# barrust/pyprobables

Measured on AMD Instinct MI355X. Metric: million keys/sec insert+lookup (Bloom m=2^28 k=7, CMS 2^20x5), higher is better.
Workload: dtype u64; 1 GPU; cfg2 Bloom m=2^28 k=7: per rank per step clear + insert 10M 16B keys + (merge) + check them; keys_per_rank=10000000, key_bytes=16, m_bits=268435456, k=7, parallelism=single GPU

## Files before the change

include/psk.h:

```cpp
#ifndef PSK_H
#define PSK_H

#include <stdint.h>

#ifdef __cplusplus
extern "C" {
#endif

typedef struct psk_sketch psk_sketch;

enum psk_status {
    PSK_OK = 0,
    PSK_EINVAL = -1,
    PSK_ENODEV = -2,
    PSK_ENOMEM = -3,
    PSK_EHIP = -4,
    PSK_ECONTRACT = -5
};

enum psk_where {
    PSK_HOST = 0,
    PSK_DEVICE = 1,
    PSK_DEVICE_BORROWED = 2
};

enum psk_layout { PSK_KEYS_FIXED = 0, PSK_KEYS_VARLEN8 = 1, PSK_KEYS_VARLEN32 = 2, PSK_KEYS_HASHES = 3 };

enum psk_query { PSK_Q_MIN = 0, PSK_Q_MEAN = 1, PSK_Q_MEANMIN = 2 };

enum psk_kind { PSK_KIND_BLOOM = 0, PSK_KIND_CBF = 1, PSK_KIND_CMS = 2 };

enum psk_opmode { PSK_OP_ADD = 0, PSK_OP_REMOVE = 1, PSK_OP_SIGNED = 2  };

enum psk_counter {
    PSK_CTR_ADDED = 0,
    PSK_CTR_REMOVED = 1,
    PSK_CTR_VIOLATIONS = 2,
    PSK_CTR_SATURATED = 3,
    PSK_CTR_ABS_BOUND = 4,
    PSK_CTR_COUNT = 8
};

const char *psk_last_error(void);
int psk_version(void);
int psk_device_count(int *count);
int psk_set_option(const char *name, int64_t value);
int psk_get_option(const char *name, int64_t *value);
int psk_sketch_set_option(psk_sketch *s, const char *name, int64_t value);
int psk_sketch_get_option(psk_sketch *s, const char *name, int64_t *value);
int psk_debug_phase_profile(psk_sketch *s, uint32_t nbuckets, uint32_t nwg, uint64_t out[12]);

uint64_t psk_bloom_table_bytes(uint64_t m_bits);
uint64_t psk_cbf_table_bytes(uint64_t m);
uint64_t psk_cms_table_bytes(uint64_t width, uint32_t depth);
int psk_bloom_create(uint64_t m_bits, uint32_t k, int device, void *ext_table, psk_sketch **out);
int psk_cbf_create(uint64_t m, uint32_t k, int device, void *ext_table, psk_sketch **out);
int psk_cms_create(uint64_t width, uint32_t depth, int device, void *ext_table, psk_sketch **out);
int psk_destroy(psk_sketch *s);
int psk_clear(psk_sketch *s, void *stream);
int psk_synchronize(psk_sketch *s, void *stream);
int psk_release_scratch(psk_sketch *s);
int psk_scratch_bytes(psk_sketch *s, uint64_t bytes[3]);
int psk_table_info(psk_sketch *s, void **dev_ptr, uint64_t *padded_bytes, uint64_t *logical_bytes);
int psk_read_table(psk_sketch *s, void *dst_host, uint64_t nbytes, void *stream);
int psk_write_table(psk_sketch *s, const void *src_host, uint64_t nbytes, void *stream);
int psk_get_counters(psk_sketch *s, int64_t out[PSK_CTR_COUNT], void *stream);
int psk_reset_counters(psk_sketch *s, void *stream);
int psk_rescan_bound(psk_sketch *s, void *stream);

int psk_bloom_add(psk_sketch *s, int layout, const void *data, const uint64_t *offsets, uint64_t n,
                  uint32_t key_len, int where, void *stream);
int psk_bloom_check(psk_sketch *s, int layout, const void *data, const uint64_t *offsets, uint64_t n,
                    uint32_t key_len, int where, uint8_t *out, void *stream);
int psk_bloom_check_bits(psk_sketch *s, int layout, const void *data, const uint64_t *offsets, uint64_t n,
                         uint32_t key_len, int where, uint64_t *out_bits, uint64_t *hits, void *stream);
int psk_bloom_check_begin(psk_sketch *s, int layout, const void *data, const uint64_t *offsets, uint64_t n, uint32_t key_len,
                          void *stream);
int psk_bloom_check_finish(psk_sketch *s, uint8_t *out_dev, void *stream);

int psk_cbf_add(psk_sketch *s, int layout, const void *data, const uint64_t *offsets, uint64_t n,
                uint32_t key_len, const uint32_t *weights, int where, void *stream);
int psk_cbf_remove(psk_sketch *s, int layout, const void *data, const uint64_t *offsets, uint64_t n,
                   uint32_t key_len, const uint32_t *weights, int where, void *stream);
int psk_cbf_check(psk_sketch *s, int layout, const void *data, const uint64_t *offsets, uint64_t n,
                  uint32_t key_len, int where, uint32_t *out, void *stream);
int psk_cbf_update_combined(psk_sketch *s, int layout, const void *data, const uint64_t *offsets, uint64_t n,
                            uint32_t key_len, const uint32_t *weights, int remove, int where, void *stream);
int psk_flush(psk_sketch *s, void *stream);
int psk_cbf_update_ordered(psk_sketch *s, int layout, const void *data, const uint64_t *offsets, uint64_t n,
                           uint32_t key_len, const int64_t *weights, int opmode, int where, uint32_t *out,
                           void *stream);

// ... 111 lines not shown
```

pyprobables_amd/_native.py:

```python

from __future__ import annotations

import ctypes as C
import os
from pathlib import Path

from .exceptions import NativeLibraryError

PSK_OK, PSK_EINVAL, PSK_ENODEV, PSK_ENOMEM, PSK_EHIP, PSK_ECONTRACT = 0, -1, -2, -3, -4, -5
HOST, DEVICE, DEVICE_BORROWED = 0, 1, 2
KEYS_FIXED, KEYS_VARLEN8, KEYS_VARLEN32, KEYS_HASHES = 0, 1, 2, 3
Q_MIN, Q_MEAN, Q_MEANMIN = 0, 1, 2
OP_ADD, OP_REMOVE, OP_SIGNED = 0, 1, 2
CTR_ADDED, CTR_REMOVED, CTR_VIOLATIONS, CTR_SATURATED, CTR_ABS_BOUND, CTR_ELS_OUT, CTR_COUNT = 0, 1, 2, 3, 4, 5, 8

LIB_PATH = Path(os.environ.get("PSK_LIB_PATH") or (Path(__file__).resolve().parent / "csrc" / "libpsk_hip.so"))

_vp, _u64, _u32, _i64, _int = C.c_void_p, C.c_uint64, C.c_uint32, C.c_int64, C.c_int
_KEYS = [_int, _vp, _vp, _u64, _u32]

PROTOTYPES = {
    "psk_last_error": (C.c_char_p, []),
    "psk_version": (_int, []),
    "psk_device_count": (_int, [C.POINTER(_int)]),
    "psk_set_option": (_int, [C.c_char_p, _i64]),
    "psk_get_option": (_int, [C.c_char_p, C.POINTER(_i64)]),
    "psk_debug_phase_profile": (_int, [_vp, _u32, _u32, C.POINTER(_u64)]),
    "psk_bloom_table_bytes": (_u64, [_u64]),
    "psk_cbf_table_bytes": (_u64, [_u64]),
    "psk_cms_table_bytes": (_u64, [_u64, _u32]),
    "psk_bloom_create": (_int, [_u64, _u32, _int, _vp, C.POINTER(_vp)]),
    "psk_cbf_create": (_int, [_u64, _u32, _int, _vp, C.POINTER(_vp)]),
    "psk_cms_create": (_int, [_u64, _u32, _int, _vp, C.POINTER(_vp)]),
    "psk_destroy": (_int, [_vp]),
    "psk_clear": (_int, [_vp, _vp]),
    "psk_synchronize": (_int, [_vp, _vp]),
    "psk_table_info": (_int, [_vp, C.POINTER(_vp), C.POINTER(_u64), C.POINTER(_u64)]),
    "psk_read_table": (_int, [_vp, _vp, _u64, _vp]),
    "psk_write_table": (_int, [_vp, _vp, _u64, _vp]),
    "psk_get_counters": (_int, [_vp, C.POINTER(_i64), _vp]),
    "psk_reset_counters": (_int, [_vp, _vp]),
    "psk_rescan_bound": (_int, [_vp, _vp]),
    "psk_sketch_set_option": (_int, [_vp, C.c_char_p, _i64]),
    "psk_sketch_get_option": (_int, [_vp, C.c_char_p, C.POINTER(_i64)]),
    "psk_bloom_add": (_int, [_vp, *_KEYS, _int, _vp]),
    "psk_bloom_check": (_int, [_vp, *_KEYS, _int, _vp, _vp]),
    "psk_bloom_check_begin": (_int, [_vp, *_KEYS, _vp]),
    "psk_bloom_check_finish": (_int, [_vp, _vp, _vp]),
    "psk_bloom_check_bits": (_int, [_vp, *_KEYS, _int, _vp, _vp, _vp]),
    "psk_cbf_add": (_int, [_vp, *_KEYS, _vp, _int, _vp]),
    "psk_cbf_remove": (_int, [_vp, *_KEYS, _vp, _int, _vp]),
    "psk_cbf_check": (_int, [_vp, *_KEYS, _int, _vp, _vp]),
    "psk_cbf_update_combined": (_int, [_vp, *_KEYS, _vp, _int, _int, _vp]),
    "psk_flush": (_int, [_vp, _vp]),
    "psk_cbf_update_ordered": (_int, [_vp, *_KEYS, _vp, _int, _int, _vp, _vp]),
    "psk_cms_add": (_int, [_vp, *_KEYS, _vp, _int, _vp]),
    "psk_cms_remove": (_int, [_vp, *_KEYS, _vp, _int, _vp]),
    "psk_cms_check": (_int, [_vp, *_KEYS, _int, _int, _vp, _vp]),
    "psk_cms_check_meanmin": (_int, [_vp, *_KEYS, _int, _i64, _vp, _vp]),
    "psk_cms_update_ordered": (_int, [_vp, *_KEYS, _vp, _int, _int, _i64, _int, _vp, _vp]),
    "psk_cms_add_running": (_int, [_vp, *_KEYS, _vp, _int, _int, _i64, _vp, _vp, _vp]),
    "psk_cms_update_running": (_int, [_vp, *_KEYS, _vp, _int, _int, _i64, _vp, _vp, _vp]),
    "psk_fnv1a_hash": (_int, [*_KEYS, _u32, _int, _vp, _int, _vp]),
    "psk_digest_chain": (_int, [_int, *_KEYS, _u32, _int, _vp, _int, _vp]),
    "psk_qf_hash": (_int, [*_KEYS, _int, _vp, _int, _vp]),
    "psk_qf_build": (_int, [_u32, _vp, _u64, _vp, _vp, _vp, _vp, _vp, _int, _vp]),
    "psk_qf_check": (_int, [_u32, _vp, _vp, _vp, _vp, *_KEYS, _int, _vp, _int, _vp]),
# ... 126 lines not shown
```

pyprobables_amd/csrc/psk_host.hpp:

```cpp
#pragma once
#include "psk_device.hpp"
#include "psk_partition.hpp"
#include "psk_part_bins.hpp"

#include <hip/hip_runtime.h>

#include <cstdarg>
#include <cstdio>
#include <cstdlib>
#include <cstring>
#include <new>
#include <type_traits>
#include <vector>

#include "../../include/psk.h"

using namespace psk;

#define PSK_HIDDEN __attribute__((visibility("hidden")))

PSK_HIDDEN int fail(int code, const char *fmt, ...);

#define HIP_TRY(expr)                                                                                   \
    do {                                                                                                \
// ... 227 lines not shown
    if (!nib_geometry(s->m, true, g)) return false;
    g->k = s->k;
    g->nwg = 256;
    g->append = 1;
    g->tile = 0;
    const double tile_keys = 2048.0 * 7.0 / (double)(s->k < 1 ? 1 : s->k);
    const double mean = (double)cap * s->k / ((double)g->nbuckets * g->nwg);
    const double runs = 2.0 * (double)cap / (tile_keys * g->nwg) + 64.0;
    const double segcap = mean / 6.0 + 0.5 * runs + 8.0 * __builtin_sqrt(mean) / 6.0 + 16.0;
    if (segcap >= (double)(1u << 24) || (double)g->nbuckets * segcap >= 4294967296.0) return false;
    g->segcap = (uint32_t)segcap;
    return true;
}

PSK_HIDDEN int raise_dyn_lds(const void *kernel, size_t bytes);

template <class K>
static int set_dyn_lds(K kernel, size_t bytes)
{
    return raise_dyn_lds((const void *)kernel, bytes);
}

template <class Pay, int KT, int NT>
static size_t scatter_lds_bytes(const PartGeom *g, uint64_t tile = 0, bool sorted = false)
{
    if (sorted) return scatter_lds_bytes<Pay, KT, NT>(g, tile, false) + 16 + 8 * (size_t)kSortBins + 18 * (size_t)PartTile<Pay, KT, NT>::TILE;
    using Tile = PartTile<Pay, KT, NT>;
    const uint32_t kk = g->k < (uint32_t)KT ? g->k : (uint32_t)KT;
    const size_t tk = tile ? (size_t)tile : (size_t)Tile::TILE;
    const size_t stage_cap = ((tk * kk + (size_t)(Tile::GS - 1) * g->nbuckets) + 3) & ~(size_t)3;
    const size_t stage_words = stage_cap + (Tile::pair ? stage_cap / Tile::GS + 4 : 0);
    return (5 * (size_t)g->nbuckets + 16 + 24 + stage_words) * 4;
}

struct ScatterTarget {
    uint32_t *cnt;
    uint4 *part;
};

#ifndef PSK_LOOKUP_FAT_SLICES
#define PSK_LOOKUP_FAT_SLICES 900
#endif
constexpr uint32_t kLookupFatSlices = PSK_LOOKUP_FAT_SLICES;
constexpr size_t kScatterLdsBudget = 160 * 1024;
constexpr size_t kScatterLdsTwoPerCu = 78 * 1024;

template <class Src>
struct src_fat512 { static constexpr bool value = std::is_same<Src, KeysFixed16>::value || std::is_same<Src, KeysFixed16Multi>::value || std::is_same<Src, KeysFixed8>::value; };

template <class Src, class Pay, int KT>
struct bins_eligible {
    static constexpr bool value = pay_bins_ok<Pay>::value && KT <= 8 && src_fat512<Src>::value;
};
constexpr size_t kBinSlackWords = 8 + 16;
struct BinsPlan {
    uint32_t tile, cap, stride, per_cu;
    size_t lds;
};
template <int KT>
static bool bins_plan(const PartGeom *g, BinsPlan *p)
{
    if (g_part_bins == 0 || g->nbuckets > (uint32_t)kBinThreads * kBinSlicesPerLane || g->nbuckets < 2) return false;
    constexpr double kSigmas = 3.5;
    const uint32_t kk = g->k < (uint32_t)KT ? g->k : (uint32_t)KT;
    p->tile = (uint32_t)kBinThreads * kBinKpt;
    const double mean = (double)p->tile * kk / (double)g->nbuckets;
    uint32_t cap = (uint32_t)(mean + kSigmas * __builtin_sqrt(mean) + 2.0);
    cap = (cap + 5) / 6 * 6;
    p->cap = cap;
    uint32_t stride = kBinHead + cap + 1;
    while (stride % 4 != 2) ++stride;
    p->stride = stride;
    p->lds = ((size_t)g->nbuckets * stride + kBinSlackWords) * 4;
    if (p->lds > kScatterLdsBudget / 2) return false;
    uint32_t per_cu = (uint32_t)(kScatterLdsBudget / p->lds);
    const uint32_t by_waves = 2048u / (uint32_t)kBinThreads;
    p->per_cu = per_cu > by_waves ? by_waves : per_cu;
    return true;
}

template <class Src, class IdxFn, class Pay, class Spill, int KT>
static int launch_scatter_bins(psk_sketch *s, const Src &src, const IdxFn &idxfn, const Pay &pay, const Spill &spill, PartGeom *g, uint64_t n,
                               hipStream_t st, uint32_t want_wgs, const BinsPlan &bp)
{
    const uint32_t kk = g->k < (uint32_t)KT ? g->k : (uint32_t)KT;
    const uint64_t tile_full = bp.tile;
    const uint64_t ntiles = (n + tile_full - 1) / tile_full;
    uint64_t nwg = 256ULL * bp.per_cu;
    if (want_wgs) nwg = want_wgs;
    if (nwg > 64u * kApplyWaves) nwg = 64u * kApplyWaves;
    if (nwg > ntiles) nwg = ntiles;
    if (nwg == 0) nwg = 1;
    const uint64_t tiles_per_wg = (ntiles + nwg - 1) / nwg;
    uint64_t tk = tile_full;
    if (g_part_even_tiles != 0 && nwg * tiles_per_wg > ntiles) {
        tk = ((n + nwg * tiles_per_wg - 1) / (nwg * tiles_per_wg) + 63) & ~63ULL;
        if (tk > tile_full) tk = tile_full;
    }
    const double mean = (double)tiles_per_wg * (double)tk * kk / (double)g->nbuckets;
    uint64_t segcap = (uint64_t)(mean / 6.0 + 0.5 * (double)tiles_per_wg + 8.0 * __builtin_sqrt(mean) / 6.0 + 16.0);
    if constexpr (pay_tile_tag<Pay>::value) {
        if (tiles_per_wg > 16) return fail(PSK_EINVAL, "lookup round of %llu keys needs %llu tiles per workgroup (max 16)",
                                           (unsigned long long)n, (unsigned long long)tiles_per_wg);
    }
    if (segcap >= (1u << 24) || (uint64_t)g->nbuckets * segcap >= (1ULL << 32))
        return fail(PSK_EINVAL, "partition round of %llu keys is too large (segments of %llu groups)", (unsigned long long)n, (unsigned long long)segcap);
    g->nwg = (uint32_t)nwg;
    g->segcap = (uint32_t)segcap;
    g->tile = (uint32_t)tk;
    g->dense = (mean / 6.0 + 0.5 * (double)tiles_per_wg) < (double)g_part_dense_groups ? 1u : 0u;
    PSK_TRY(ensure(s->s_part, (uint64_t)g->nbuckets * nwg * segcap * 16 + 256));
    PSK_TRY(ensure(s->s_cnt, (uint64_t)g->nbuckets * nwg * 4 + 128));
    auto kern = k_part_bins<Src, IdxFn, Pay, Spill, KT, kBinKpt>;
    PSK_TRY(set_dyn_lds(kern, bp.lds));
    hipLaunchKernelGGL(kern, dim3((unsigned)nwg), dim3(kBinThreads), bp.lds, st, src, idxfn, pay, spill, *g, (uint32_t)n, bp.cap, bp.stride,
                       (uint32_t *)s->s_cnt.p, (uint4 *)s->s_part.p);
    HIP_TRY(hipGetLastError());
    return PSK_OK;
}
template <class Src, class IdxFn, class Pay, class Spill, int KT, int NT>
static int launch_scatter_nt(psk_sketch *s, const Src &src, const IdxFn &idxfn, const Pay &pay, const Spill &spill, PartGeom *g,
                             uint64_t n, hipStream_t st, uint32_t want_wgs, const ScatterTarget *fixed = nullptr)
{
    if constexpr (bins_eligible<Src, Pay, KT>::value) {
        BinsPlan bp;
        if (!fixed && n < (1ULL << 31) && bins_plan<KT>(g, &bp)) return launch_scatter_bins<Src, IdxFn, Pay, Spill, KT>(s, src, idxfn, pay, spill, g, n, st, want_wgs, bp);
    }
// ... 301 lines not shown
```

pyprobables_amd/csrc/psk_part_bins.hpp:

```cpp
#pragma once
#include "psk_partition.hpp"

namespace psk {

#ifndef PSK_BINS_NT
#define PSK_BINS_NT 768
#endif
constexpr int kBinThreads = PSK_BINS_NT;
constexpr int kBinMinWaves = kBinThreads <= 512 ? 4 : (kBinThreads <= 768 ? 6 : 8);
#ifndef PSK_BINS_KPT
#define PSK_BINS_KPT 2
#endif
constexpr int kBinKpt = PSK_BINS_KPT;
constexpr int kBinSlicesPerLane = 2;

template <class Pay>
struct pay_bins_ok { static constexpr bool value = false; };
template <>
struct pay_bins_ok<PayNone> { static constexpr bool value = true; };
template <>
struct pay_bins_ok<PayTileTag> { static constexpr bool value = true; };
template <>
struct pay_bins_ok<PayWeightSmall> { static constexpr bool value = true; };

constexpr uint32_t kBinHead = 2;
template <class Src, class IdxFn, class Pay, class Spill, int KT, int KPT>
__global__ __launch_bounds__(kBinThreads, kBinMinWaves) void k_part_bins(Src src, IdxFn idxfn, Pay pay, Spill spill, PartGeom g, uint32_t n, uint32_t cap,
                                                              uint32_t stride, uint32_t *segcnt, uint4 *buckets)
{
    constexpr int NT = kBinThreads;
    extern __shared__ __attribute__((aligned(16))) uint32_t smem[];
    char *lds = reinterpret_cast<char *>(smem);
    const uint32_t B = g.nbuckets;
    constexpr bool kExactK = KT != 8;
    const uint32_t k = kExactK ? (uint32_t)KT : g.k;
    const uint32_t mask = (1u << g.shift) - 1;
    const uint32_t tk = g.tile;
    const uint32_t ntiles = (n + tk - 1) / tk;
    const uint32_t last = n ? n - 1 : 0;
    const uint32_t stride4 = stride * 4u;
    const uint32_t lg_slices = 31u - (uint32_t)__builtin_clz(B);
    const uint32_t full4 = (cap + kBinHead) * 4u;
    constexpr uint32_t kCnt = 4;

    uint32_t L = 1;
    while (2 * L * B <= (uint32_t)NT) L *= 2;
    constexpr int kSlicesPerLane = kBinSlicesPerLane;
    const uint32_t sub = B <= (uint32_t)NT ? threadIdx.x % L : 0u;
    uint32_t myb[kSlicesPerLane], cur[kSlicesPerLane];
    uint4 *seg[kSlicesPerLane];
#pragma unroll
    for (int s = 0; s < kSlicesPerLane; ++s) {
        myb[s] = B <= (uint32_t)NT ? (s == 0 && threadIdx.x / L < B ? threadIdx.x / L : ~0u) : threadIdx.x + (uint32_t)s * NT;
        if (myb[s] >= B) myb[s] = ~0u;
        cur[s] = 0;
        seg[s] = buckets + (seg_index(g, 0, blockIdx.x) + (myb[s] == ~0u ? 0u : myb[s])) * g.segcap;
    }
    for (uint32_t b = threadIdx.x; b < B; b += NT) *reinterpret_cast<uint32_t *>(lds + b * stride4 + kCnt) = kBinHead * 4u;

    const uint32_t dbg = kBenchKnobs ? g.dbg : 0u;
    unsigned long long *t_acc = reinterpret_cast<unsigned long long *>(lds + (size_t)B * stride4 + 32);
    unsigned long long t_prev = 0;
    const bool t_lane = (dbg & 32) && (threadIdx.x == 0 || threadIdx.x == NT - 64);
    const uint32_t t_base = threadIdx.x == 0 ? 0u : 4u;
    if ((dbg & 32) && threadIdx.x < 8) t_acc[threadIdx.x] = 0;
#define PSK_BIN_TICK(ph)                                                 \
    if (t_lane) {                                                        \
        const unsigned long long t_now = __builtin_readcyclecounter();   \
        t_acc[t_base + (ph)] += t_now - t_prev;                          \
        t_prev = t_now;                                                  \
    }
    uint32_t fold = 0;
    constexpr bool WP = pay_weighted_plain<Pay>::value;
    typename Src::Key kcur[KPT];
    uint32_t wcur[WP ? KPT : 1];
    long long tally_s = 0;
    unsigned long long tally_a = 0;
    uint32_t tally_b = 0;
    {
        const uint32_t b0 = blockIdx.x * tk;
#pragma unroll
        for (int q = 0; q < KPT; ++q) {
            const uint32_t i = b0 + (uint32_t)q * NT + threadIdx.x;
            kcur[q] = src.load(i < last ? i : last);
            if constexpr (WP) wcur[q] = pay(i < last ? i : last, 0);
        }
    }
    lds_barrier();
    if (t_lane) t_prev = __builtin_readcyclecounter();

    uint32_t ordinal = ~0u;
    for (uint32_t tile = blockIdx.x; tile < ntiles; tile += gridDim.x) {
        ++ordinal;
        const uint32_t base = tile * tk;
        const uint32_t tile_end = base + tk < n ? base + tk : n;
        if constexpr (PSK_EXP_PRIO == 1) __builtin_amdgcn_s_setprio(0);
#pragma unroll
        for (int q = 0; q < KPT; ++q) {
            const uint32_t i = base + (uint32_t)q * NT + threadIdx.x;
            if ((uint32_t)q * NT < tk && i < tile_end) {
                uint32_t val[KT], bin[KT];
                uint32_t wfield = 0, wbig = 0, wq = 0;
                if constexpr (WP) {
                    wq = wcur[q];
                    if (pay.tally) {
                        const long long v = pay.weights_signed ? (long long)(int32_t)wq : (long long)wq;
                        tally_s += v;
                        tally_a += (unsigned long long)(v < 0 ? -v : v);
// ... 43 lines not shown
                    if ((uint32_t)j < k) {
                        at[j] = __umul24(bin[j], stride4);
                        r4[j] = atomicAdd(reinterpret_cast<uint32_t *>(lds + at[j] + kCnt), 4u);
                    }
                }
#pragma unroll
                for (int j = 0; j < KT; ++j) {
                    if ((uint32_t)j < k) {
                        worst = r4[j] > worst ? r4[j] : worst;
                        *reinterpret_cast<uint32_t *>(lds + at[j] + (r4[j] < full4 ? r4[j] : full4)) = WP ? (val[j] | wfield) : val[j];
                    }
                }
                if constexpr (WP) {
                    if (wbig) {
#pragma unroll
                        for (int j = 0; j < KT; ++j)
                            if ((uint32_t)j < k) spill((bin[j] << g.shift) | val[j], wq);
                    }
                }
                if (worst >= full4) {
#pragma unroll
                    for (int j = 0; j < KT; ++j)
                        if ((uint32_t)j < k && r4[j] >= full4) {
                            if constexpr (pay_tile_tag<Pay>::value) spill((bin[j] << g.shift) | val[j], tile);
                            else if constexpr (WP) { if (!wbig) spill((bin[j] << g.shift) | val[j], wq); }
                            else spill((bin[j] << g.shift) | val[j], 0u);
                        }
                }
            }
        }
        {
            const uint32_t nb = (tile + gridDim.x) * tk;
#pragma unroll
            for (int q = 0; q < KPT; ++q) {
                const uint32_t i = nb + (uint32_t)q * NT + threadIdx.x;
                kcur[q] = src.load(i < last ? i : last);
                if constexpr (WP) wcur[q] = pay(i < last ? i : last, 0);
            }
        }
        if (dbg & 2) {
            if (fold == 0x12345u) segcnt[0] = fold;
            continue;
        }
        PSK_BIN_TICK(0);
        lds_barrier();
        PSK_BIN_TICK(1);
        if constexpr (PSK_EXP_PRIO == 1) __builtin_amdgcn_s_setprio(3);

        const uint32_t t0 = pay_tile_tag<Pay>::value ? (ordinal & 3u) << 2 : 0u, t1 = pay_tile_tag<Pay>::value ? ordinal & 12u : 0u;
#pragma unroll
        for (int s = 0; s < kSlicesPerLane; ++s) {
            const uint32_t b = myb[s];
            if (b == ~0u) continue;
            const char *bin = lds + b * stride4;
            const uint32_t c4 = *reinterpret_cast<const uint32_t *>(bin + kCnt);
            const uint32_t c = ((c4 < full4 ? c4 : full4) >> 2) - kBinHead;
            const uint32_t whole = c / 6u, rem = c - 6u * whole, ngroups = whole + (rem ? 1u : 0u);
            const uint2 *e = reinterpret_cast<const uint2 *>(bin + kBinHead * 4u);
            uint4 *out = seg[s] + cur[s];
            if (cur[s] + ngroups <= g.segcap) {
                const uint32_t hi0 = (3u | t0) << 28, hi1 = (3u | t1) << 28;
                for (uint32_t gq = sub; gq < whole; gq += L) {
                    const uint2 a0 = e[3 * gq], a1 = e[3 * gq + 1], a2 = e[3 * gq + 2];
                    uint4 o;
                    o.x = a0.x | (a0.y << 20);
                    o.y = (a0.y >> 12) | (a1.x << 8) | hi0;
                    o.z = a1.y | (a2.x << 20);
                    o.w = (a2.x >> 12) | (a2.y << 8) | hi1;
                    if (!(dbg & 1)) out[gq] = o;
                }
                if (rem && sub == (whole & (L - 1))) {
                    const uint2 a0 = e[3 * whole], a1 = e[3 * whole + 1], a2 = e[3 * whole + 2];
                    uint32_t f[6] = {a0.x, a0.y, a1.x, a1.y, a2.x, a2.y};
#pragma unroll
                    for (int x = 1; x < 6; ++x)
                        if ((uint32_t)x >= rem) f[x] = WP ? 0u : mask;
                    const uint32_t n0 = rem < 3u ? rem : 3u, n1 = rem - n0;
                    uint4 o;
                    o.x = f[0] | (f[1] << 20);
                    o.y = (f[1] >> 12) | (f[2] << 8) | ((n0 | t0) << 28);
                    o.z = f[3] | (f[4] << 20);
                    o.w = (f[4] >> 12) | (f[5] << 8) | ((n1 | t1) << 28);
                    if (!(dbg & 1)) out[whole] = o;
                }
            } else {
                for (uint32_t gq = sub; gq < ngroups; gq += L) {
                    const uint2 a0 = e[3 * gq], a1 = e[3 * gq + 1], a2 = e[3 * gq + 2];
                    uint32_t f[6] = {a0.x, a0.y, a1.x, a1.y, a2.x, a2.y};
                    const uint32_t left = c - 6u * gq, nv = left < 6u ? left : 6u;
#pragma unroll
                    for (int x = 1; x < 6; ++x)
                        if ((uint32_t)x >= nv) f[x] = WP ? 0u : mask;
                    const uint32_t n0 = nv < 3u ? nv : 3u, n1 = nv - n0;
                    if (cur[s] + gq < g.segcap) {
                        uint4 o;
                        o.x = f[0] | (f[1] << 20);
                        o.y = (f[1] >> 12) | (f[2] << 8) | ((n0 | t0) << 28);
                        o.z = f[3] | (f[4] << 20);
                        o.w = (f[4] >> 12) | (f[5] << 8) | ((n1 | t1) << 28);
                        out[gq] = o;
                    } else {
#pragma unroll
                        for (int x = 0; x < 6; ++x)
                            if ((uint32_t)x < nv) {
                                if constexpr (pay_tile_tag<Pay>::value) spill((b << g.shift) | f[x], tile);
                                else if constexpr (WP) spill((b << g.shift) | (f[x] & mask), f[x] >> 15);
                                else spill((b << g.shift) | f[x], 0u);
                            }
                    }
                }
            }
            cur[s] += ngroups;
        }
#pragma unroll
        for (int s = 0; s < kSlicesPerLane; ++s)
            if (myb[s] != ~0u && sub == 0) *reinterpret_cast<uint32_t *>(lds + myb[s] * stride4 + kCnt) = kBinHead * 4u;
#pragma unroll
        for (int q = 0; q < KPT; ++q) {
            Src::pin(kcur[q]);
            if constexpr (WP) asm volatile("" : "+v"(wcur[q]));
        }
        PSK_BIN_TICK(2);
        lds_barrier();
        PSK_BIN_TICK(3);
    }
    if (t_lane) {
        unsigned long long *prof = reinterpret_cast<unsigned long long *>(segcnt + (size_t)g.nbuckets * g.nwg);
        for (int ph = 0; ph < 4; ++ph) atomicAdd(prof + 1 + t_base + ph, t_acc[t_base + ph]);
        if (threadIdx.x == 0) atomicAdd(prof, 1ULL);
    }
#undef PSK_BIN_TICK
    if constexpr (WP) {
        if (pay.tally) {
            for (int o = 32; o > 0; o >>= 1) {
                tally_s += __shfl_down(tally_s, o);
                tally_a += __shfl_down(tally_a, o);
                tally_b += __shfl_down(tally_b, o);
            }
            unsigned long long *red = reinterpret_cast<unsigned long long *>(smem);
            if ((threadIdx.x & 63) == 0) {
                red[3 * (threadIdx.x >> 6)] = (unsigned long long)tally_s;
                red[3 * (threadIdx.x >> 6) + 1] = tally_a;
                red[3 * (threadIdx.x >> 6) + 2] = tally_b;
            }
            lds_barrier();
            if (threadIdx.x == 0) {
                unsigned long long ss = 0, aa = 0, bb = 0;
                for (int w = 0; w < NT / 64; ++w) { ss += red[3 * w]; aa += red[3 * w + 1]; bb += red[3 * w + 2]; }
                pay.tally[blockIdx.x] = make_ulonglong4(ss, aa, bb, 0ULL);
            }
        }
    }
#pragma unroll
    for (int s = 0; s < kSlicesPerLane; ++s)
        if (myb[s] != ~0u && sub == 0) segcnt[(uint64_t)myb[s] * g.nwg + blockIdx.x] = cur[s] < g.segcap ? cur[s] : g.segcap;
}

}
```

pyprobables_amd/csrc/psk_part_bloom_add.hip:

```cpp
#include "psk_host.hpp"

static_assert(kBloomApplyCtrWords == PSK_CTR_COUNT, "k_bloom_apply's store mode zeroes the whole counter block");

int PSK_VARIANT(bloom_add_partitioned)(psk_sketch *s, const Batch &b, hipStream_t st, bool *done)
{
    *done = false;
    if (!part_wanted(s, b.n, s->k)) return PSK_OK;
    PartGeom g;
    if (!part_slices(s->m, 20, 7, &g, 16384)) return PSK_OK;
    g.k = s->k;
    PartGeom g1;
    uint32_t sub_bits = 0;
    if (two_level_geometry(g, &g1, &sub_bits)) {
        PSK_TRY(clear_materialize(s, st));
        const uint64_t round_keys = part_round_keys_two_level(s, b.n, s->k);
        for (uint64_t start = 0; start < b.n; start += round_keys) {
            const uint64_t cnt = b.n - start < round_keys ? b.n - start : round_keys;
            const Batch sub = sub_batch(b, start, cnt);
            bool handled = false;
            SpillBloomOr spill{(uint32_t *)s->table};
            PSK_TRY(with_part_source(sub, &handled, [&](auto src) {
                using Src = decltype(src);
                return with_kt<Src>(s->k, [&](auto kt) {
                    constexpr int KT = decltype(kt)::value;
                    return launch_scatter<Src, IdxBloomWide<kTuPow2>, PayZero, SpillBloomOr, KT>(s, src, IdxBloomWide<kTuPow2>{s->md}, PayZero{},
                                                                                              spill, &g1, cnt, st);
                });
            }));
            if (!handled) return PSK_OK;
            PartGeom g2 = g;
            PSK_TRY((split_level2<0, SpillBloomOr>(s, g1, &g2, sub_bits, cnt * (uint64_t)s->k, spill, st)));
            const size_t lds = (size_t)1 << (g2.shift - 3);
            PSK_TRY(set_dyn_lds(k_bloom_apply, lds));
            hipLaunchKernelGGL(k_bloom_apply, dim3(g2.nbuckets), dim3(kApplyThreads), lds, st, (uint32_t *)s->table, s->padded_bytes / 4,
                               g2, (const uint32_t *)s->s_cnt2.p, (const uint4 *)s->s_part2.p, BloomApplyStore{});
            HIP_TRY(hipGetLastError());
        }
        *done = true;
        return PSK_OK;
    }
    if (g.nbuckets > (uint32_t)kPartMaxBuckets) return PSK_OK;
    const uint64_t round_keys = part_round_keys_big_table(s, b.n, s->k, PayNone::group, s->padded_bytes);
    BloomApplyStore first;
    if (s->clear_pending) {
        const uint64_t probes = (b.n < round_keys ? b.n : round_keys) * (uint64_t)s->k;
        if (probes < (1ULL << 32) - 2) {
            const uint64_t oldcap = s->s_spill.cap;
            PSK_TRY(ensure(s->s_spill, (2 + probes) * 4));
            if (s->s_spill.cap != oldcap) HIP_TRY(hipMemsetAsync(s->s_spill.p, 0, 8, st));
            first = BloomApplyStore{1u, (const uint32_t *)s->s_spill.p, (uint32_t)probes, s->ctr};
        }
    }
    if (!first.on) PSK_TRY(clear_materialize(s, st));
    for (uint64_t start = 0; start < b.n; start += round_keys) {
        const uint64_t cnt = b.n - start < round_keys ? b.n - start : round_keys;
// ... 24 lines not shown
```

pyprobables_amd/csrc/psk_partition.hpp:

```cpp
#pragma once
#include <type_traits>
#include "psk_device.hpp"

#ifndef PSK_BENCH_KNOBS
#define PSK_BENCH_KNOBS 0
#endif

namespace psk {

constexpr bool kBenchKnobs = PSK_BENCH_KNOBS != 0;
constexpr int kPartThreads = 512;
constexpr int kPartProbes = 32;
constexpr int kPartMaxBuckets = 2048;
constexpr int kPartScanPerThread = 4;
constexpr bool kPartPipeline = true;
constexpr bool kPartHash32 = true;
constexpr uint32_t kNibShift = 18;
constexpr uint32_t kGeomNoSortBit = 0x40000000u;
constexpr int kSortSub = 16;
constexpr int kSortBins = 64 * kSortSub;
constexpr uint32_t kPadProbe = 0xFFFFFFFFu;
#ifndef PSK_EXP_PRIO
#define PSK_EXP_PRIO 1
#endif
// ... 1176 lines not shown
        }
        return *reinterpret_cast<const uint4 *>(tab + gw);
    }
    uint4 t = make_uint4(0, 0, 0, 0);
    if (gw + 0 < tab_words) t.x = tab[gw + 0];
    if (gw + 1 < tab_words) t.y = tab[gw + 1];
    if (gw + 2 < tab_words) t.z = tab[gw + 2];
    return t;
}

constexpr int kSliceLoads = 8;
__device__ __forceinline__ void load_slice(uint32_t *smem, const uint32_t *tab, uint64_t tab_words, uint64_t w0, uint32_t slice_words)
{
    const bool nt = tab_words >= kNtTableWords;
    for (uint32_t wb = threadIdx.x * 4; wb < slice_words; wb += kApplyThreads * 4 * kSliceLoads) {
        uint4 t[kSliceLoads];
#pragma unroll
        for (int u = 0; u < kSliceLoads; ++u) {
            const uint32_t w = wb + (uint32_t)u * kApplyThreads * 4;
            t[u] = w < slice_words ? slice_piece(tab, tab_words, w0, w, nt) : make_uint4(0, 0, 0, 0);
        }
#pragma unroll
        for (int u = 0; u < kSliceLoads; ++u) {
            const uint32_t w = wb + (uint32_t)u * kApplyThreads * 4;
            if (w < slice_words) *reinterpret_cast<uint4 *>(smem + w) = t[u];
        }
    }
}

template <int DEPTH = kApplyDepth, class F4>
__device__ __forceinline__ void for_each_group(const uint4 *buckets, const uint32_t *segcnt, const PartGeom &g, uint32_t b,
                                               const uint4 pad, F4 f4)
{
    for_each_batch<DEPTH>(buckets, segcnt, g, b, pad, [&](const uint4 (&q)[DEPTH]) {
#pragma unroll
        for (int d = 0; d < DEPTH; ++d) f4(q[d]);
    });
}

template <class Pre, class Post>
__device__ __forceinline__ void for_each_group_padded(const uint4 *buckets, const uint32_t *segcnt, const PartGeom &g, uint32_t b,
                                                      const uint4 pad, Pre pre, Post post)
{
    for_each_batch<kApplyDepth>(buckets, segcnt, g, b, pad, [&](const uint4 (&q)[kApplyDepth]) {
        uint4 w[kApplyDepth];
#pragma unroll
        for (int d = 0; d < kApplyDepth; ++d) w[d] = pre(q[d]);
#pragma unroll
        for (int d = 0; d < kApplyDepth; ++d) post(q[d], w[d]);
    });
}

constexpr uint32_t kBloomApplyCtrWords = 8;
struct BloomApplyStore {
    uint32_t on = 0;
    const uint32_t *spill = nullptr;
    uint32_t spill_cap = 0;
    long long *ctr = nullptr;
};
static __global__ __launch_bounds__(kApplyThreads) void k_bloom_apply(uint32_t *tab, uint64_t tab_words, PartGeom g,
                                                               const uint32_t *segcnt, const uint4 *buckets, BloomApplyStore sm)
{
    extern __shared__ __attribute__((aligned(16))) uint32_t smem[];
    const uint32_t b = blockIdx.x;
    const uint32_t slice_words = 1u << (g.shift - 5);
    for (uint32_t w = threadIdx.x; w < slice_words; w += kApplyThreads) smem[w] = 0;
    __syncthreads();
    auto half = [&](uint32_t lo, uint32_t hi) {
        const unsigned long long h = ((unsigned long long)hi << 32) | lo;
        const uint32_t nv = hi >> 28;
        if (nv > 0) { const uint32_t x = (uint32_t)h & 0xFFFFFu; atomicOr(&smem[x >> 5], 1u << (x & 31)); }
        if (nv > 1) { const uint32_t x = (uint32_t)(h >> 20) & 0xFFFFFu; atomicOr(&smem[x >> 5], 1u << (x & 31)); }
        if (nv > 2) { const uint32_t x = (uint32_t)(h >> 40) & 0xFFFFFu; atomicOr(&smem[x >> 5], 1u << (x & 31)); }
    };
    for_each_group(buckets, segcnt, g, b, make_uint4(0, 0, 0, 0), [&](const uint4 q) { half(q.x, q.y); half(q.z, q.w); });
    if (sm.on) {
        const uint32_t nsp = sm.spill[0] < sm.spill_cap ? sm.spill[0] : sm.spill_cap;
        const uint32_t lmask = (1u << g.shift) - 1u;
        for (uint32_t i = threadIdx.x; i < nsp; i += kApplyThreads) {
            const uint32_t x = sm.spill[2 + i];
            if ((x >> g.shift) == b) atomicOr(&smem[(x & lmask) >> 5], 1u << (x & 31));
        }
    }
    __syncthreads();
    const uint64_t w0 = (uint64_t)b * slice_words;
    const bool nt = tab_words >= kNtTableWords;
    typedef unsigned int nt_u32x4 __attribute__((ext_vector_type(4)));
    if (sm.on) {
        for (uint32_t w = threadIdx.x * 4; w < slice_words; w += kApplyThreads * 4) {
            const uint64_t gw = w0 + w;
            const uint4 v = *reinterpret_cast<const uint4 *>(smem + w);
            if (gw + 3 < tab_words) {
                if (nt) {
                    nt_u32x4 x;
                    x.x = v.x; x.y = v.y; x.z = v.z; x.w = v.w;
                    __builtin_nontemporal_store(x, reinterpret_cast<nt_u32x4 *>(tab + gw));
                } else {
                    *reinterpret_cast<uint4 *>(tab + gw) = v;
                }
            } else {
                const uint32_t vv[4] = {v.x, v.y, v.z, v.w};
                for (uint32_t e = 0; e < 4; ++e)
                    if (gw + e < tab_words) tab[gw + e] = vv[e];
            }
        }
        if (b == gridDim.x - 1)
            for (uint64_t gw = (uint64_t)gridDim.x * slice_words + threadIdx.x; gw < tab_words; gw += kApplyThreads) tab[gw] = 0;
        if (b == 0 && threadIdx.x < kBloomApplyCtrWords) sm.ctr[threadIdx.x] = 0;
        if (threadIdx.x == 0) {
            uint32_t *hdr = const_cast<uint32_t *>(sm.spill);
            if (atomicAdd(hdr + 1, 1u) == gridDim.x - 1) {
                hdr[0] = 0;
                hdr[1] = 0;
            }
        }
        return;
    }
    constexpr int kFold = 4;
    for (uint32_t wb = threadIdx.x * 4; wb < slice_words; wb += kApplyThreads * 4 * kFold) {
        uint4 t[kFold], add[kFold];
        bool full[kFold];
#pragma unroll
        for (int u = 0; u < kFold; ++u) {
            const uint32_t w = wb + (uint32_t)u * kApplyThreads * 4;
            const uint64_t gw = w0 + w;
            full[u] = w < slice_words && gw + 3 < tab_words;
            add[u] = w < slice_words ? *reinterpret_cast<const uint4 *>(smem + w) : make_uint4(0, 0, 0, 0);
            t[u] = make_uint4(0, 0, 0, 0);
            if (full[u] && (add[u].x | add[u].y | add[u].z | add[u].w)) {
                if (nt) {
                    const nt_u32x4 v = __builtin_nontemporal_load(reinterpret_cast<const nt_u32x4 *>(tab + gw));
                    t[u] = make_uint4(v.x, v.y, v.z, v.w);
                } else {
                    t[u] = *reinterpret_cast<const uint4 *>(tab + gw);
                }
            }
        }
#pragma unroll
        for (int u = 0; u < kFold; ++u) {
            const uint32_t w = wb + (uint32_t)u * kApplyThreads * 4;
            const uint64_t gw = w0 + w;
            if (!(add[u].x | add[u].y | add[u].z | add[u].w)) continue;
            if (full[u]) {
                t[u].x |= add[u].x; t[u].y |= add[u].y; t[u].z |= add[u].z; t[u].w |= add[u].w;
                if (nt) {
                    nt_u32x4 v;
                    v.x = t[u].x; v.y = t[u].y; v.z = t[u].z; v.w = t[u].w;
                    __builtin_nontemporal_store(v, reinterpret_cast<nt_u32x4 *>(tab + gw));
                } else {
                    *reinterpret_cast<uint4 *>(tab + gw) = t[u];
                }
            } else if (w < slice_words) {
                const uint32_t aa[4] = {add[u].x, add[u].y, add[u].z, add[u].w};
                for (uint32_t e = 0; e < 4; ++e)
                    if (gw + e < tab_words && aa[e]) tab[gw + e] |= aa[e];
            }
        }
    }
}

static __global__ __launch_bounds__(kApplyThreads) void k_bloom_test(const uint32_t *tab, uint64_t tab_words, PartGeom g,
// ... 56 lines not shown
                                                                   unsigned long long *miss_ctr, uint8_t *out, uint64_t n)
{
    uint32_t nmiss = 0;
    extern __shared__ __attribute__((aligned(16))) uint32_t smem[];
    const uint32_t b = blockIdx.x;
    {
        const uintptr_t a0 = (uintptr_t)out, a1 = a0 + n;
        const uintptr_t m0 = (a0 + 15) & ~(uintptr_t)15, m1 = a1 & ~(uintptr_t)15;
        if (m0 < m1) {
            const uint64_t pieces = (m1 - m0) >> 4, per = (pieces + gridDim.x - 1) / gridDim.x;
            const uint64_t lo = (uint64_t)b * per, hi = lo + per < pieces ? lo + per : pieces;
            const uint4 ones = make_uint4(0x01010101u, 0x01010101u, 0x01010101u, 0x01010101u);
            uint4 *mid = reinterpret_cast<uint4 *>(out + (m0 - a0));
            for (uint64_t i = lo + threadIdx.x; i < hi; i += kApplyThreads) mid[i] = ones;
            if (b == 0) {
                if (threadIdx.x < (uint32_t)(m0 - a0)) out[threadIdx.x] = 1;
                if (threadIdx.x < (uint32_t)(a1 - m1)) out[(m1 - a0) + threadIdx.x] = 1;
            }
        } else if (b == 0) {
            for (uint64_t i = threadIdx.x; i < n; i += kApplyThreads) out[i] = 1;
        }
    }
    const uint32_t slice_words = 1u << (g.shift - 5);
    const uint64_t w0 = (uint64_t)b * slice_words;
    const uint32_t mycnt = lane_segment_count(segcnt, g, b);
    load_slice(smem, tab, tab_words, w0, slice_words);
    __syncthreads();
    for_each_batch_at<kFlagDepth>(buckets, segcnt, g, b, make_uint4(0, 0, 0, 0), [&](const uint4 (&q)[kFlagDepth], const uint64_t (&)[kFlagDepth],
                                                                                   const uint32_t (&wg)[kFlagDepth]) {
        uint32_t f[kFlagDepth][6], w[kFlagDepth][6];
#pragma unroll
        for (int d = 0; d < kFlagDepth; ++d) {
            f[d][0] = q[d].x & 0xFFFFFu;
            f[d][1] = __builtin_amdgcn_alignbit(q[d].y, q[d].x, 20) & 0xFFFFFu;
            f[d][2] = (q[d].y >> 8) & 0xFFFFFu;
            f[d][3] = q[d].z & 0xFFFFFu;
            f[d][4] = __builtin_amdgcn_alignbit(q[d].w, q[d].z, 20) & 0xFFFFFu;
            f[d][5] = (q[d].w >> 8) & 0xFFFFFu;
#pragma unroll
            for (int e = 0; e < 6; ++e) w[d][e] = smem[f[d][e] >> 5];
        }
#pragma unroll
        for (int d = 0; d < kFlagDepth; ++d) {
            uint32_t clear = 0;
#pragma unroll
            for (int e = 0; e < 6; ++e) clear |= (((w[d][e] >> (f[d][e] & 31)) & 1u) ^ 1u) << e;
            const uint32_t n0 = (q[d].y >> 28) & 3u, n1 = (q[d].w >> 28) & 3u;
            const uint32_t valid = ((1u << n0) - 1u) | (((1u << n1) - 1u) << 3);
            clear &= valid;
            if (clear) {
                nmiss += (uint32_t)__builtin_popcount(clear);
                const uint32_t ordinal = (q[d].y >> 30) | ((q[d].w >> 30) << 2);
                tileflag[ordinal * g.nwg + wg[d]] = gen;
                tileflag[-1] = gen;
            }
        }
    }, mycnt);
    if (miss_ctr) {
        for (int o = 32; o > 0; o >>= 1) nmiss += __shfl_down(nmiss, o);
        __syncthreads();
        if ((threadIdx.x & 63) == 0) smem[threadIdx.x >> 6] = nmiss;
        __syncthreads();
        if (threadIdx.x == 0) {
            unsigned long long t = 0;
            for (int w = 0; w < kApplyWaves; ++w) t += smem[w];
            if (t) atomicAdd(miss_ctr, t);
        }
    }
}

constexpr int kResolveThreads = 1024;
struct LookupPublish {
    unsigned long long *tally = nullptr;
    volatile unsigned long long *pin = nullptr;
    unsigned long long units = 0, scheme = 0;
};
template <class Src, bool POW2>
__global__ __launch_bounds__(kResolveThreads) void k_bloom_flag_resolve(Src src, const uint32_t *tab, Mod md, uint32_t k, const uint32_t *tileflag, uint32_t gen,
                                                                       uint32_t tile, uint64_t n, uint8_t *out, LookupPublish pub)
{
    if (pub.tally && blockIdx.x == 0 && threadIdx.x == 0) {
        pub.pin[1] = pub.units;
        pub.pin[2] = pub.scheme;
        pub.pin[0] = pub.tally[0];
        pub.pin[3] = pub.pin[3] + 1;
        pub.tally[0] = 0;
    }
    if (tileflag[-1] != gen) return;
    const uint64_t ntiles = (n + tile - 1) / tile;
    BloomCheck<POW2> op{tab, md, k, out};
    for (uint64_t t0 = 0; t0 * gridDim.x + blockIdx.x < ntiles; t0 += 64) {
        const uint64_t mine = (t0 + (threadIdx.x & 63)) * gridDim.x + blockIdx.x;
        unsigned long long todo = __ballot(mine < ntiles && tileflag[mine < ntiles ? mine : 0] == gen);
        while (todo) {
            const uint32_t l = (uint32_t)__builtin_ctzll(todo);
            todo &= todo - 1;
            const uint64_t t = (t0 + l) * gridDim.x + blockIdx.x, base = t * tile;
            const uint32_t cnt = (uint32_t)(n - base < tile ? n - base : tile);
            for (uint32_t j = threadIdx.x; j < cnt; j += kResolveThreads) {
                const uint64_t i = base + j;
                const typename Src::Key key = src.load(i);
                typename BloomCheck<POW2>::State st = op.begin(i);
                for_each_hash(src, key, i, k, [&](uint32_t jj, uint64_t h) { op.apply(st, jj, h); });
                op.end(st, i);
            }
        }
// ... 184 lines not shown
```

Baseline: 59950 Mkeys/s.

## Carry partial bin groups across tiles instead of flushing short groups

```diff
diff --git a/include/psk.h b/include/psk.h
--- a/include/psk.h
+++ b/include/psk.h
@@ -38,6 +38,7 @@
     PSK_CTR_VIOLATIONS = 2,
     PSK_CTR_SATURATED = 3,
     PSK_CTR_ABS_BOUND = 4,
+    PSK_CTR_SPILLED = 7,
     PSK_CTR_COUNT = 8
 };
 
diff --git a/pyprobables_amd/_native.py b/pyprobables_amd/_native.py
--- a/pyprobables_amd/_native.py
+++ b/pyprobables_amd/_native.py
@@ -12,7 +12,7 @@
 KEYS_FIXED, KEYS_VARLEN8, KEYS_VARLEN32, KEYS_HASHES = 0, 1, 2, 3
 Q_MIN, Q_MEAN, Q_MEANMIN = 0, 1, 2
 OP_ADD, OP_REMOVE, OP_SIGNED = 0, 1, 2
-CTR_ADDED, CTR_REMOVED, CTR_VIOLATIONS, CTR_SATURATED, CTR_ABS_BOUND, CTR_ELS_OUT, CTR_COUNT = 0, 1, 2, 3, 4, 5, 8
+CTR_ADDED, CTR_REMOVED, CTR_VIOLATIONS, CTR_SATURATED, CTR_ABS_BOUND, CTR_ELS_OUT, CTR_SPILLED, CTR_COUNT = 0, 1, 2, 3, 4, 5, 7, 8
 
 LIB_PATH = Path(os.environ.get("PSK_LIB_PATH") or (Path(__file__).resolve().parent / "csrc" / "libpsk_hip.so"))
 
diff --git a/pyprobables_amd/csrc/psk_host.hpp b/pyprobables_amd/csrc/psk_host.hpp
--- a/pyprobables_amd/csrc/psk_host.hpp
+++ b/pyprobables_amd/csrc/psk_host.hpp
@@ -303,6 +303,9 @@
 struct bins_eligible {
     static constexpr bool value = pay_bins_ok<Pay>::value && KT <= 8 && src_fat512<Src>::value;
 };
+#ifndef PSK_BINS_CARRY_GROUP
+#define PSK_BINS_CARRY_GROUP 1
+#endif
 constexpr size_t kBinSlackWords = 8 + 16;
 struct BinsPlan {
     uint32_t tile, cap, stride, per_cu;
@@ -318,12 +321,17 @@
     const double mean = (double)p->tile * kk / (double)g->nbuckets;
     uint32_t cap = (uint32_t)(mean + kSigmas * __builtin_sqrt(mean) + 2.0);
     cap = (cap + 5) / 6 * 6;
-    p->cap = cap;
-    uint32_t stride = kBinHead + cap + 1;
-    while (stride % 4 != 2) ++stride;
-    p->stride = stride;
-    p->lds = ((size_t)g->nbuckets * stride + kBinSlackWords) * 4;
-    if (p->lds > kScatterLdsBudget / 2) return false;
+    auto plan = [&](uint32_t c) {
+        uint32_t stride = kBinHead + c + 1;
+        while (stride % 4 != 2) ++stride;
+        const size_t lds = ((size_t)g->nbuckets * stride + kBinSlackWords) * 4;
+        if (lds > kScatterLdsBudget / 2) return false;
+        p->cap = c;
+        p->stride = stride;
+        p->lds = lds;
+        return true;
+    };
+    if (!(PSK_BINS_CARRY_GROUP && plan(cap + 6)) && !plan(cap)) return false;
     uint32_t per_cu = (uint32_t)(kScatterLdsBudget / p->lds);
     const uint32_t by_waves = 2048u / (uint32_t)kBinThreads;
     p->per_cu = per_cu > by_waves ? by_waves : per_cu;
diff --git a/pyprobables_amd/csrc/psk_part_bins.hpp b/pyprobables_amd/csrc/psk_part_bins.hpp
--- a/pyprobables_amd/csrc/psk_part_bins.hpp
+++ b/pyprobables_amd/csrc/psk_part_bins.hpp
@@ -24,6 +24,21 @@
 struct pay_bins_ok<PayWeightSmall> { static constexpr bool value = true; };
 
 constexpr uint32_t kBinHead = 2;
+template <bool WP>
+__device__ __forceinline__ uint4 bin_short_group(const uint2 a0, const uint2 a1, const uint2 a2, uint32_t nv, uint32_t mask, uint32_t t0, uint32_t t1)
+{
+    uint32_t f[6] = {a0.x, a0.y, a1.x, a1.y, a2.x, a2.y};
+#pragma unroll
+    for (int x = 1; x < 6; ++x)
+        if ((uint32_t)x >= nv) f[x] = WP ? 0u : mask;
+    const uint32_t n0 = nv < 3u ? nv : 3u, n1 = nv - n0;
+    uint4 o;
+    o.x = f[0] | (f[1] << 20);
+    o.y = (f[1] >> 12) | (f[2] << 8) | ((n0 | t0) << 28);
+    o.z = f[3] | (f[4] << 20);
+    o.w = (f[4] >> 12) | (f[5] << 8) | ((n1 | t1) << 28);
+    return o;
+}
 template <class Src, class IdxFn, class Pay, class Spill, int KT, int KPT>
 __global__ __launch_bounds__(kBinThreads, kBinMinWaves) void k_part_bins(Src src, IdxFn idxfn, Pay pay, Spill spill, PartGeom g, uint32_t n, uint32_t cap,
                                                               uint32_t stride, uint32_t *segcnt, uint4 *buckets)
@@ -48,12 +63,14 @@
     constexpr int kSlicesPerLane = kBinSlicesPerLane;
     const uint32_t sub = B <= (uint32_t)NT ? threadIdx.x % L : 0u;
     uint32_t myb[kSlicesPerLane], cur[kSlicesPerLane];
+    uint32_t carry[kSlicesPerLane];
     uint4 *seg[kSlicesPerLane];
 #pragma unroll
     for (int s = 0; s < kSlicesPerLane; ++s) {
         myb[s] = B <= (uint32_t)NT ? (s == 0 && threadIdx.x / L < B ? threadIdx.x / L : ~0u) : threadIdx.x + (uint32_t)s * NT;
         if (myb[s] >= B) myb[s] = ~0u;
         cur[s] = 0;
+        carry[s] = 0;
         seg[s] = buckets + (seg_index(g, 0, blockIdx.x) + (myb[s] == ~0u ? 0u : myb[s])) * g.segcap;
     }
     for (uint32_t b = threadIdx.x; b < B; b += NT) *reinterpret_cast<uint32_t *>(lds + b * stride4 + kCnt) = kBinHead * 4u;
@@ -203,11 +220,13 @@
         for (int s = 0; s < kSlicesPerLane; ++s) {
             const uint32_t b = myb[s];
             if (b == ~0u) continue;
-            const char *bin = lds + b * stride4;
+            char *bin = lds + b * stride4;
             const uint32_t c4 = *reinterpret_cast<const uint32_t *>(bin + kCnt);
             const uint32_t c = ((c4 < full4 ? c4 : full4) >> 2) - kBinHead;
-            const uint32_t whole = c / 6u, rem = c - 6u * whole, ngroups = whole + (rem ? 1u : 0u);
-            const uint2 *e = reinterpret_cast<const uint2 *>(bin + kBinHead * 4u);
+            const uint32_t whole = c / 6u, rem = c - 6u * whole;
+            const bool tail = pay_tile_tag<Pay>::value && whole == 0 && carry[s] != 0;
+            const uint32_t ngroups = whole + (tail ? 1u : 0u);
+            uint2 *e = reinterpret_cast<uint2 *>(bin + kBinHead * 4u);
             uint4 *out = seg[s] + cur[s];
             if (cur[s] + ngroups <= g.segcap) {
                 const uint32_t hi0 = (3u | t0) << 28, hi1 = (3u | t1) << 28;
@@ -220,52 +239,45 @@
                     o.w = (a2.x >> 12) | (a2.y << 8) | hi1;
                     if (!(dbg & 1)) out[gq] = o;
                 }
-                if (rem && sub == (whole & (L - 1))) {
+                if constexpr (pay_tile_tag<Pay>::value) {
+                    if (tail && sub == 0 && !(dbg & 1)) out[0] = bin_short_group<WP>(e[0], e[1], e[2], rem, mask, t0, t1);
+                }
+                if (rem && whole && sub == (whole & (L - 1))) {
+                    __builtin_amdgcn_wave_barrier();
                     const uint2 a0 = e[3 * whole], a1 = e[3 * whole + 1], a2 = e[3 * whole + 2];
-                    uint32_t f[6] = {a0.x, a0.y, a1.x, a1.y, a2.x, a2.y};
-#pragma unroll
-                    for (int x = 1; x < 6; ++x)
-                        if ((uint32_t)x >= rem) f[x] = WP ? 0u : mask;
-                    const uint32_t n0 = rem < 3u ? rem : 3u, n1 = rem - n0;
-                    uint4 o;
-                    o.x = f[0] | (f[1] << 20);
-                    o.y = (f[1] >> 12) | (f[2] << 8) | ((n0 | t0) << 28);
-                    o.z = f[3] | (f[4] << 20);
-                    o.w = (f[4] >> 12) | (f[5] << 8) | ((n1 | t1) << 28);
-                    if (!(dbg & 1)) out[whole] = o;
-                }
+                    e[0] = a0;
+                    e[1] = a1;
+                    e[2] = a2;
+                }
+                carry[s] = tail ? 0u : rem;
+                cur[s] += ngroups;
             } else {
-                for (uint32_t gq = sub; gq < ngroups; gq += L) {
+                const uint32_t nall = whole + (rem ? 1u : 0u);
+                for (uint32_t gq = sub; gq < nall; gq += L) {
                     const uint2 a0 = e[3 * gq], a1 = e[3 * gq + 1], a2 = e[3 * gq + 2];
-                    uint32_t f[6] = {a0.x, a0.y, a1.x, a1.y, a2.x, a2.y};
                     const uint32_t left = c - 6u * gq, nv = left < 6u ? left : 6u;
-#pragma unroll
-                    for (int x = 1; x < 6; ++x)
-                        if ((uint32_t)x >= nv) f[x] = WP ? 0u : mask;
-                    const uint32_t n0 = nv < 3u ? nv : 3u, n1 = nv - n0;
                     if (cur[s] + gq < g.segcap) {
-                        uint4 o;
-                        o.x = f[0] | (f[1] << 20);
-                        o.y = (f[1] >> 12) | (f[2] << 8) | ((n0 | t0) << 28);
-                        o.z = f[3] | (f[4] << 20);
-                        o.w = (f[4] >> 12) | (f[5] << 8) | ((n1 | t1) << 28);
-                        out[gq] = o;
+                        out[gq] = bin_short_group<WP>(a0, a1, a2, nv, mask, t0, t1);
                     } else {
+                        const uint32_t f[6] = {a0.x, a0.y, a1.x, a1.y, a2.x, a2.y};
 #pragma unroll
                         for (int x = 0; x < 6; ++x)
                             if ((uint32_t)x < nv) {
-                                if constexpr (pay_tile_tag<Pay>::value) spill((b << g.shift) | f[x], tile);
-                                else if constexpr (WP) spill((b << g.shift) | (f[x] & mask), f[x] >> 15);
+                                if constexpr (pay_tile_tag<Pay>::value) {
+                                    spill((b << g.shift) | f[x], tile);
+                                    if (ordinal) spill((b << g.shift) | f[x], tile - gridDim.x);
+                                } else if constexpr (WP) spill((b << g.shift) | (f[x] & mask), f[x] >> 15);
                                 else spill((b << g.shift) | f[x], 0u);
                             }
                     }
                 }
-            }
-            cur[s] += ngroups;
+                carry[s] = 0;
+                cur[s] += nall;
+            }
         }
 #pragma unroll
         for (int s = 0; s < kSlicesPerLane; ++s)
-            if (myb[s] != ~0u && sub == 0) *reinterpret_cast<uint32_t *>(lds + myb[s] * stride4 + kCnt) = kBinHead * 4u;
+            if (myb[s] != ~0u && sub == 0) *reinterpret_cast<uint32_t *>(lds + myb[s] * stride4 + kCnt) = (kBinHead + carry[s]) * 4u;
 #pragma unroll
         for (int q = 0; q < KPT; ++q) {
             Src::pin(kcur[q]);
@@ -274,6 +286,28 @@
         PSK_BIN_TICK(2);
         lds_barrier();
         PSK_BIN_TICK(3);
+    }
+    if (ordinal != ~0u) {
+        const uint32_t t0 = pay_tile_tag<Pay>::value ? (ordinal & 3u) << 2 : 0u, t1 = pay_tile_tag<Pay>::value ? ordinal & 12u : 0u;
+#pragma unroll
+        for (int s = 0; s < kSlicesPerLane; ++s) {
+            if (myb[s] == ~0u || sub != 0 || carry[s] == 0) continue;
+            const uint2 *e = reinterpret_cast<const uint2 *>(lds + myb[s] * stride4 + kBinHead * 4u);
+            const uint2 a0 = e[0], a1 = e[1], a2 = e[2];
+            if (cur[s] < g.segcap) {
+                if (!(dbg & 1)) seg[s][cur[s]] = bin_short_group<WP>(a0, a1, a2, carry[s], mask, t0, t1);
+            } else {
+                const uint32_t f[6] = {a0.x, a0.y, a1.x, a1.y, a2.x, a2.y};
+#pragma unroll
+                for (int x = 0; x < 6; ++x)
+                    if ((uint32_t)x < carry[s]) {
+                        if constexpr (pay_tile_tag<Pay>::value) spill((myb[s] << g.shift) | f[x], ordinal * gridDim.x + blockIdx.x);
+                        else if constexpr (WP) spill((myb[s] << g.shift) | (f[x] & mask), f[x] >> 15);
+                        else spill((myb[s] << g.shift) | f[x], 0u);
+                    }
+            }
+            cur[s] += 1;
+        }
     }
     if (t_lane) {
         unsigned long long *prof = reinterpret_cast<unsigned long long *>(segcnt + (size_t)g.nbuckets * g.nwg);
@@ -288,6 +322,7 @@
                 tally_a += __shfl_down(tally_a, o);
                 tally_b += __shfl_down(tally_b, o);
             }
+            lds_barrier();
             unsigned long long *red = reinterpret_cast<unsigned long long *>(smem);
             if ((threadIdx.x & 63) == 0) {
                 red[3 * (threadIdx.x >> 6)] = (unsigned long long)tally_s;
diff --git a/pyprobables_amd/csrc/psk_part_bloom_add.hip b/pyprobables_amd/csrc/psk_part_bloom_add.hip
--- a/pyprobables_amd/csrc/psk_part_bloom_add.hip
+++ b/pyprobables_amd/csrc/psk_part_bloom_add.hip
@@ -1,6 +1,7 @@
 #include "psk_host.hpp"
 
 static_assert(kBloomApplyCtrWords == PSK_CTR_COUNT, "k_bloom_apply's store mode zeroes the whole counter block");
+static_assert(kBloomApplyCtrSpilled == PSK_CTR_SPILLED, "... and leaves the length of pass 1's spill list in this slot");
 
 int PSK_VARIANT(bloom_add_partitioned)(psk_sketch *s, const Batch &b, hipStream_t st, bool *done)
 {
diff --git a/pyprobables_amd/csrc/psk_partition.hpp b/pyprobables_amd/csrc/psk_partition.hpp
--- a/pyprobables_amd/csrc/psk_partition.hpp
+++ b/pyprobables_amd/csrc/psk_partition.hpp
@@ -1252,6 +1252,7 @@
 }
 
 constexpr uint32_t kBloomApplyCtrWords = 8;
+constexpr uint32_t kBloomApplyCtrSpilled = 7;
 struct BloomApplyStore {
     uint32_t on = 0;
     const uint32_t *spill = nullptr;
@@ -1274,8 +1275,10 @@
         if (nv > 2) { const uint32_t x = (uint32_t)(h >> 40) & 0xFFFFFu; atomicOr(&smem[x >> 5], 1u << (x & 31)); }
     };
     for_each_group(buckets, segcnt, g, b, make_uint4(0, 0, 0, 0), [&](const uint4 q) { half(q.x, q.y); half(q.z, q.w); });
+    uint32_t spilled = 0;
     if (sm.on) {
-        const uint32_t nsp = sm.spill[0] < sm.spill_cap ? sm.spill[0] : sm.spill_cap;
+        spilled = sm.spill[0];
+        const uint32_t nsp = spilled < sm.spill_cap ? spilled : sm.spill_cap;
         const uint32_t lmask = (1u << g.shift) - 1u;
         for (uint32_t i = threadIdx.x; i < nsp; i += kApplyThreads) {
             const uint32_t x = sm.spill[2 + i];
@@ -1306,7 +1309,7 @@
         }
         if (b == gridDim.x - 1)
             for (uint64_t gw = (uint64_t)gridDim.x * slice_words + threadIdx.x; gw < tab_words; gw += kApplyThreads) tab[gw] = 0;
-        if (b == 0 && threadIdx.x < kBloomApplyCtrWords) sm.ctr[threadIdx.x] = 0;
+        if (b == 0 && threadIdx.x < kBloomApplyCtrWords) sm.ctr[threadIdx.x] = threadIdx.x == kBloomApplyCtrSpilled ? (long long)spilled : 0;
         if (threadIdx.x == 0) {
             uint32_t *hdr = const_cast<uint32_t *>(sm.spill);
             if (atomicAdd(hdr + 1, 1u) == gridDim.x - 1) {
@@ -1469,6 +1472,7 @@
                 nmiss += (uint32_t)__builtin_popcount(clear);
                 const uint32_t ordinal = (q[d].y >> 30) | ((q[d].w >> 30) << 2);
                 tileflag[ordinal * g.nwg + wg[d]] = gen;
+                if (ordinal) tileflag[(ordinal - 1u) * g.nwg + wg[d]] = gen;
                 tileflag[-1] = gen;
             }
         }
```

Result: faster. 60870 Mkeys/s, median of 6 (+1.5%).
